# rhofield/rho-tts

Measured on AMD Instinct MI355X. Metric: audio-sec/wall-sec (RTF) Qwen3-TTS-1.7B batch=32, higher is better.
Workload: dtype bf16; 1 GPU; Qwen3-TTS-1.7B bf16, batch 32/GPU, 30-s reference clone, 10-word sentences (44 frames each), sampling=top-k 50 T 0.9, seeded synthetic weights; value counts delivered (post-processed) audio; global_batch=32, parallelism=dp1

## Files before the change

### include/rho_tts_amd_debug.h

```cpp
#ifndef RHO_TTS_AMD_DEBUG_H
#define RHO_TTS_AMD_DEBUG_H

#include "rho_tts_amd.h"

#ifdef __cplusplus
extern "C" {
#endif

RT_API int rt_profile_enable(rt_model* m, int32_t on);
RT_API int rt_profile_read(rt_model* m, int64_t* n_launches, double* total_ms, double* total_bytes);
RT_API int rt_profile_read_class(rt_model* m, int32_t cls, int64_t* n_launches, double* total_ms, double* total_bytes);

RT_API int rt_debug_gemm(rt_ctx* ctx, const void* d_a, int32_t a_is_f32, int64_t M, int32_t cin, int32_t taps, int32_t tap_stride,
                         int32_t tap_offset, int32_t rows_out, int32_t rows_in, const void* d_w_bf16, int32_t N,
                         const float* d_bias, int32_t act, float* d_out, int32_t mode, int32_t split_k);
RT_API int rt_debug_attention(rt_ctx* ctx, const float* d_q, int32_t M, int32_t heads, int32_t kv_heads, int32_t head_dim,
                              const int32_t* d_row_slot, const int32_t* d_row_pos, int32_t window, const void* d_k, const void* d_v,
                              int32_t slots, int32_t max_pos, void* d_out_bf16);
RT_API int rt_debug_attention_planes(rt_ctx* ctx, const float* d_q, int32_t M, int32_t heads, int32_t kv_heads, int32_t head_dim,
                                     const int32_t* d_row_slot, const int32_t* d_row_pos, int32_t window, const void* d_k_hi,
                                     const void* d_k_lo, const void* d_v_hi, const void* d_v_lo, int32_t slots, int32_t max_pos,
                                     float* d_out_f32);
RT_API int rt_debug_gemm_col(rt_ctx* ctx, const void* d_a_bf16, int32_t M, int32_t K, const void* d_w_bf16, int32_t N, int32_t epi, int32_t split,
                             int32_t row_off, int32_t nt, const float* d_rowsq, int32_t rowsq_n, float eps, const float* d_bias,
// ... 119 lines not shown
                             const rt_debug_epi* e2, int32_t pair_mode);

RT_API int rt_debug_enc_conv0(rt_ctx* ctx, const float* d_pcm, int64_t T, int32_t C, int32_t K, const float* d_w, const float* d_bias, float* d_x,
                              void* d_hi, void* d_lo);
RT_API int rt_debug_rvq(rt_ctx* ctx, const float* d_sem, float* d_aco, int32_t T, int32_t D, int32_t K, int32_t Q, const void* const* h_cbT,
                        int32_t* d_codes);
RT_API int rt_debug_stats_pool(rt_ctx* ctx, const float* d_x, int32_t T, int32_t C, float* d_out);
RT_API int rt_debug_gemv_f32(rt_ctx* ctx, const float* d_W, const float* d_b_or_NULL, const float* d_x, int32_t N, int32_t K, int32_t relu,
                             float* d_y);
RT_API int rt_debug_voice_encode_stages(rt_model* m, const float* h_pcm, int64_t n_samples, int32_t max_frames, float* h_feats, float* h_tf,
                                        float* h_emb, float* h_sem, float* h_aco, int32_t* h_codes, int32_t* h_n_frames,
                                        float* h_speaker_embed);

RT_API int rt_debug_tune(int32_t code, int32_t arg);
RT_API int rt_debug_col_row_blocks(int32_t n_cu, int32_t M, int32_t N, int32_t epi, int32_t split);
RT_API int rt_bench_gemm_col(rt_ctx* ctx, int32_t M, int32_t N, int32_t K, int32_t a_norm, int32_t epi, int32_t n_mats, int32_t iters,
                             double* avg_us, int64_t* stamps8);
RT_API int rt_bench_stt_gather(rt_ctx* ctx, int32_t layers, int32_t rows, int32_t heads, int32_t max_pos, int32_t head_dim, int32_t prefix, int32_t step,
                               int32_t iters, double* us_ranged, double* us_uniform);
RT_API int rt_bench_launch(rt_ctx* ctx, int32_t grid_wgs, int32_t n, int32_t use_graph, int32_t reps, double* us_per_launch);
RT_API int rt_bench_grid_barrier(rt_ctx* ctx, int32_t wgs, int32_t threads, int32_t n, int32_t mode, double* us_per_barrier, int32_t* aborted);
RT_API int rt_bench_sample(rt_ctx* ctx, const float* d_logits, int32_t M, int32_t V, const rt_sampling* sp, int32_t iters, double* avg_us,
                           int64_t* stamps8);
RT_API int rt_bench_attention_fused(rt_ctx* ctx, int32_t M, int32_t heads, int32_t kv_heads, int32_t head_dim, int32_t prefix_len, int32_t own_len,
                                    int32_t shared, int32_t layers, int32_t iters, double* avg_us);
RT_API int rt_bench_gemm_skinny(rt_ctx* ctx, int32_t M, int32_t N, int32_t K, int32_t split_k, int32_t n_mats, int32_t iters,
                                double* avg_us, int32_t* used_split);

#ifdef __cplusplus
}
// ... 3 lines not shown
```

### rho_tts_amd/csrc/debug.hip

```cpp
#include <algorithm>
#include <vector>

#include "kernels.h"

namespace {
__global__ void k_touch(float* p, int n) {
    const int i = blockIdx.x * blockDim.x + threadIdx.x;
    if (i < n) p[i] = p[i] * 1.0001f + 1.0f;
}
template <int MODE>
__global__ void k_bench_barrier(unsigned* bar, int n, float* buf) {
    const int i = blockIdx.x * blockDim.x + threadIdx.x;
    const int j = (i + blockDim.x) % (gridDim.x * blockDim.x);
    float acc = buf[i];
    for (int e = 1; e <= n; ++e) {
        if (MODE == 2) st_agent(buf + i, acc + 1.0f); else buf[i] = acc + 1.0f;
        if (!grid_barrier<MODE>(bar, gridDim.x, (unsigned)e, 1u << 20)) return;
        acc = MODE == 2 ? ld_agent(buf + j) : buf[j];
        if (acc != (float)e && i == 0) bar[2] = 1u;
    }
    buf[i] = acc;
}
template <int P>
__global__ void k_bench_pair(unsigned* flags, int n, float* buf, unsigned* bar) {
// ... 13 lines not shown
                while (__hip_atomic_load(flags + mate * 32, __ATOMIC_ACQUIRE, __HIP_MEMORY_SCOPE_AGENT) < (unsigned)e)
                    if (++spins > (1u << 22)) { bar[1] = 1u; break; }
            }
            __syncthreads();
            if (bar[1]) return;
            if (t < 512 && ld_agent(theirs + t) != (float)e) bar[2] = 1u;
        }
    }
}
__global__ void k_iota64(int64_t* p, int n) {
    const int i = blockIdx.x * blockDim.x + threadIdx.x;
    if (i < n) p[i] = i;
}

template <typename T>
__global__ void k_tile_rows(const T* __restrict__ src, int M, int K, int row_off, T* __restrict__ dst) {
    const int64_t n = (int64_t)M * K;
    for (int64_t i = (int64_t)blockIdx.x * blockDim.x + threadIdx.x; i < n; i += (int64_t)gridDim.x * blockDim.x) {
        const int m = (int)(i / K), k = (int)(i % K);
        dst[tile_off(row_off + m, k, K)] = src[i];
    }
}
template <typename T>
__global__ void k_untile_rows(const T* __restrict__ src, int M, int K, int row_off, T* __restrict__ dst) {
    const int64_t n = (int64_t)M * K;
    for (int64_t i = (int64_t)blockIdx.x * blockDim.x + threadIdx.x; i < n; i += (int64_t)gridDim.x * blockDim.x) {
        const int m = (int)(i / K), k = (int)(i % K);
        dst[i] = src[tile_off(row_off + m, k, K)];
    }
}
}

#define RT_KNOB_DEFINE(base, name, def, lo, hi, doc) rt_knob name{def};
RT_KNOBS(RT_KNOB_DEFINE)
RT_KNOB_ARG(RT_KNOB_DEFINE)
#undef RT_KNOB_DEFINE
std::atomic<int> g_tune_epoch{0};
namespace {
struct KnobRow { int base, lo, hi; rt_knob* knob; };
#define RT_KNOB_ROW(base, name, def, lo, hi, doc) {base, lo, hi, &name},
const KnobRow kKnobs[] = {RT_KNOBS(RT_KNOB_ROW)};
const KnobRow kKnobArg[] = {RT_KNOB_ARG(RT_KNOB_ROW)};
#undef RT_KNOB_ROW
// ... 82 lines not shown
}

int rt_debug_gemm_col(rt_ctx* ctx, const void* d_a_bf16, int32_t M, int32_t K, const void* d_w_bf16, int32_t N, int32_t epi, int32_t split,
                      int32_t row_off, int32_t nt, const float* d_rowsq, int32_t rowsq_n, float eps, const float* d_bias, const float* d_scale,
                      float* d_x, const float* d_next_norm_w, void* d_next_bf16, float* d_rowsq_out, void* d_act_bf16) {
    if (!ctx || !d_a_bf16 || !d_w_bf16 || M < 1 || M > 128 || K < 32 || K % 32 || N < 1 || row_off < 0 || row_off % 16)
        return rt_fail(ctx, RT_ERR_INVALID, "rt_debug_gemm_col: bad argument (1 <= M <= 128, K %% 32 == 0, row_off %% 16 == 0)");
    if (epi < COL_STORE || epi > COL_SILU) return rt_fail(ctx, RT_ERR_INVALID, "rt_debug_gemm_col: epi %d", epi);
    if ((epi != COL_SILU && !d_x) || (epi == COL_SILU && (!d_act_bf16 || N % 32)) || (epi == COL_RESID && !d_rowsq_out))
        return rt_fail(ctx, RT_ERR_INVALID, "rt_debug_gemm_col: missing output for epilogue %d", epi);
    CtxLock g(ctx);
    RT_HIP(ctx, hipSetDevice(ctx->device));
    const int No = epi == COL_SILU ? N / 2 : N;
    if (split <= 0) split = epi == COL_SILU ? col_split_silu(N, ctx->n_cu) : col_split_for(N, ctx->n_cu);
    const int rows = (row_off + M + 31) / 32 * 32;
    bf16_t *w16 = nullptr, *a_t = nullptr, *next_t = nullptr, *act_t = nullptr;
    float *x_t = nullptr, *rowsq_all = nullptr, *rowsq_out_all = nullptr;
    int rc = RT_OK;
    auto cleanup = [&]() {
        (void)hipStreamSynchronize(ctx->stream);
        for (void* p : {(void*)w16, (void*)a_t, (void*)next_t, (void*)act_t, (void*)x_t, (void*)rowsq_all, (void*)rowsq_out_all}) if (p) (void)hipFree(p);
    };
#define DBG_HIP(expr) do { hipError_t _e = (expr); if (_e != hipSuccess) { cleanup(); return rt_fail(ctx, rt_hip_status(_e), "%s failed: %s", #expr, hipGetErrorString(_e)); } } while (0)
    DBG_HIP(hipMalloc((void**)&w16, packed16_bytes(N, K)));
    DBG_HIP(hipMalloc((void**)&a_t, (size_t)rows * K * 2));
    DBG_HIP(hipMemsetAsync(a_t, 0, (size_t)rows * K * 2, ctx->stream));
    PackedW pw;
    pw.N = N; pw.K = K;
    rc = launch_pack_weight16(ctx, (const bf16_t*)d_w_bf16, N, K, w16, &pw);
    const int nb = 256;
    hipLaunchKernelGGL((k_tile_rows<bf16_t>), dim3(nb), dim3(256), 0, ctx->stream, (const bf16_t*)d_a_bf16, M, K, row_off, a_t);
    const int n_part = (N + 15) / 16 * split;
    ColArgs c;
    c.A = a_t; c.M = M; c.K = K; c.epi = epi; c.split = split; c.row_off = row_off; c.nt = nt ? 1 : 0; c.eps = eps;
    c.bias = d_bias; c.scale = d_scale; c.ldc = No;
    if (d_rowsq) {
        DBG_HIP(hipMalloc((void**)&rowsq_all, (size_t)rows * rowsq_n * 4));
        DBG_HIP(hipMemsetAsync(rowsq_all, 0, (size_t)rows * rowsq_n * 4, ctx->stream));
        DBG_HIP(hipMemcpyAsync(rowsq_all + (size_t)row_off * rowsq_n, d_rowsq, (size_t)M * rowsq_n * 4, hipMemcpyDeviceToDevice, ctx->stream));
        c.post_scale = 1; c.rowsq = rowsq_all; c.rowsq_n = rowsq_n;
    }
    if (epi == COL_STORE) {
        c.out = d_x - (size_t)row_off * No;
    } else if (epi == COL_RESID) {
        DBG_HIP(hipMalloc((void**)&x_t, (size_t)rows * No * 4));
        DBG_HIP(hipMemsetAsync(x_t, 0, (size_t)rows * No * 4, ctx->stream));
        hipLaunchKernelGGL((k_tile_rows<float>), dim3(nb), dim3(256), 0, ctx->stream, (const float*)d_x, M, No, row_off, x_t);
        DBG_HIP(hipMalloc((void**)&rowsq_out_all, (size_t)rows * n_part * 4));
        DBG_HIP(hipMemsetAsync(rowsq_out_all, 0, (size_t)rows * n_part * 4, ctx->stream));
        c.out = x_t; c.rowsq_out = rowsq_out_all; c.rowsq_out_n = n_part;
        if (d_next_bf16) {
            DBG_HIP(hipMalloc((void**)&next_t, (size_t)rows * No * 2));
            DBG_HIP(hipMemsetAsync(next_t, 0, (size_t)rows * No * 2, ctx->stream));
            c.next_bf16 = next_t; c.next_norm_w = d_next_norm_w;
        }
    } else {
        DBG_HIP(hipMalloc((void**)&act_t, (size_t)rows * No * 2));
        DBG_HIP(hipMemsetAsync(act_t, 0, (size_t)rows * No * 2, ctx->stream));
        c.out_bf16 = act_t;
    }
    const int blk = (M > 64 && g_col_rows128) ? 128 : (g_col_rows64 ? 64 : 32);
    for (int r0 = 0; r0 < M && !rc; r0 += blk) {
        ColArgs a = c;
        a.M = std::min(blk, M - r0);
        a.row_off = row_off + r0;
        rc = launch_gemm_col(ctx, a, pw);
    }
    if (!rc && epi == COL_RESID) {
        hipLaunchKernelGGL((k_untile_rows<float>), dim3(nb), dim3(256), 0, ctx->stream, (const float*)x_t, M, No, row_off, d_x);
        if (next_t) hipLaunchKernelGGL((k_untile_rows<bf16_t>), dim3(nb), dim3(256), 0, ctx->stream, (const bf16_t*)next_t, M, No, row_off, (bf16_t*)d_next_bf16);
        DBG_HIP(hipMemcpyAsync(d_rowsq_out, rowsq_out_all + (size_t)row_off * n_part, (size_t)M * n_part * 4, hipMemcpyDeviceToDevice, ctx->stream));
    }
    if (!rc && epi == COL_SILU)
        hipLaunchKernelGGL((k_untile_rows<bf16_t>), dim3(nb), dim3(256), 0, ctx->stream, (const bf16_t*)act_t, M, No, row_off, (bf16_t*)d_act_bf16);
    if (!rc) DBG_HIP(hipGetLastError());
#undef DBG_HIP
    cleanup();
    return rc;
}

int rt_debug_attention_fused(rt_ctx* ctx, const float* d_qkv, int32_t M, int32_t heads, int32_t kv_heads, int32_t head_dim, const float* d_q_norm_w,
                             const float* d_k_norm_w, float eps, const float* d_cos, const float* d_sin, const int32_t* d_row_slot,
                             const int32_t* d_row_pos, int32_t pos_add, void* d_k, void* d_v, int32_t slots, int32_t max_pos,
                             int32_t prefix_slot, int32_t prefix_len, void* d_out_bf16) {
    if (!ctx || !d_qkv || !d_cos || !d_sin || !d_k || !d_v || !d_out_bf16 || M < 1)
        return rt_fail(ctx, RT_ERR_INVALID, "rt_debug_attention_fused: null argument");
    if (prefix_slot >= slots || prefix_len < 0 || prefix_len > max_pos) return rt_fail(ctx, RT_ERR_INVALID, "rt_debug_attention_fused: bad prefix");
    CtxLock g(ctx);
    RT_HIP(ctx, hipSetDevice(ctx->device));
// ... 117 lines not shown
    RT_HIP(ctx, bufs.alloc(out, sizeof(GatherSrc) * (size_t)n_src));
    RT_HIP(ctx, hipMemcpy(*out, h.data(), sizeof(GatherSrc) * (size_t)n_src, hipMemcpyHostToDevice));
    return RT_OK;
}
int dbg_finish(rt_ctx* ctx, int rc) {
    const hipError_t se = hipStreamSynchronize(ctx->stream);
    if (rc) return rc;
    RT_HIP(ctx, se);
    return RT_OK;
}
template <typename T>
int dbg_tile_in(rt_ctx* ctx, DbgBufs& bufs, const T* rows_rm, int rows, int H, T** tiled) {
    const size_t pad = (size_t)(rows + 15) / 16 * 16;
    RT_HIP(ctx, bufs.alloc(tiled, pad * H * sizeof(T)));
    RT_HIP(ctx, hipMemsetAsync(*tiled, 0, pad * H * sizeof(T), ctx->stream));
    hipLaunchKernelGGL((k_tile_rows<T>), dim3(256), dim3(256), 0, ctx->stream, rows_rm, rows, H, 0, *tiled);
    RT_HIP(ctx, hipGetLastError());
    return RT_OK;
}
template <typename T>
int dbg_tile_out(rt_ctx* ctx, const T* tiled, int rows, int H, T* rows_rm) {
    hipLaunchKernelGGL((k_untile_rows<T>), dim3(256), dim3(256), 0, ctx->stream, tiled, rows, H, 0, rows_rm);
    RT_HIP(ctx, hipGetLastError());
    return RT_OK;
}
int dbg_read_i32(rt_ctx* ctx, const int32_t* d, int n, std::vector<int32_t>& h) {
    h.assign((size_t)n, 0);
    RT_HIP(ctx, hipStreamSynchronize(ctx->stream));
    RT_HIP(ctx, hipMemcpy(h.data(), d, (size_t)n * 4, hipMemcpyDeviceToHost));
    return RT_OK;
}
}
}

int rt_debug_add_rmsnorm(rt_ctx* ctx, float* d_x, int32_t M, int32_t H, const float* d_slabs, int32_t n_slabs, const float* d_slab_bias,
                         const float* d_scale, const float* d_w, float eps, void* d_out_bf16, float* d_out_f32) {
    if (!ctx || !d_x || M < 1 || H < 1 || n_slabs < 0 || (n_slabs > 0 && !d_slabs))
// ... 267 lines not shown
        if (code >= r.base + r.lo && code <= r.base + r.hi) {
            *r.knob = code - r.base;
            if (r.base == kKnobArg[0].base && arg >= kKnobArg[0].lo && arg <= kKnobArg[0].hi) *kKnobArg[0].knob = arg;
            ++g_tune_epoch;
            return RT_OK;
        }
    return RT_ERR_INVALID;
}

int rt_debug_col_row_blocks(int32_t n_cu, int32_t M, int32_t N, int32_t epi, int32_t split) {
    if (n_cu < 1 || M < 1 || M > 128 || N < 1 || epi < COL_STORE || epi > COL_SILU || (epi == COL_SILU && N % 32) || split > 4 || split == 3) return -1;
    std::shared_lock<std::shared_mutex> plan(g_tune_mu);
    bool x_form = false;
    const int wg = col_workgroups(n_cu, M, N, epi, split, &x_form);
    return col_row_blocks(n_cu, M, wg, x_form);
}

int rt_bench_gemm_skinny(rt_ctx* ctx, int32_t M, int32_t N, int32_t K, int32_t split_k, int32_t n_mats, int32_t iters, double* avg_us,
                         int32_t* used_split) {
    if (!ctx || !avg_us || M < 1 || M > 64 || N < 32 || K < 16 || K % 16 || n_mats < 1 || iters < 1) return rt_fail(ctx, RT_ERR_INVALID, "rt_bench_gemm_skinny: bad argument");
    CtxLock g(ctx);
    RT_HIP(ctx, hipSetDevice(ctx->device));
    const size_t pb = packed_bytes(N, K);
    bf16_t* wbuf = nullptr;
    bf16_t* a = nullptr;
    float* out = nullptr;
    if (split_k < 1) split_k = skinny_pick_split(M, N, K, ctx->n_cu);
    if (used_split) *used_split = split_k;
    RT_HIP(ctx, hipMalloc((void**)&wbuf, pb * n_mats));
    RT_HIP(ctx, hipMalloc((void**)&a, (size_t)M * K * 2));
// ... 372 lines not shown
```

### rho_tts_amd/csrc/gemm_col.hip

```cpp
#include <hip/hip_ext.h>

#include "kernels.h"

namespace {

typedef __attribute__((ext_vector_type(8))) __bf16 bf8_t;
typedef __attribute__((ext_vector_type(8))) short s8_t;
typedef __attribute__((ext_vector_type(16))) float f16_t;
typedef __attribute__((ext_vector_type(4))) float f4_t;
typedef __attribute__((ext_vector_type(4))) int i4_t;

__device__ __forceinline__ f16_t mfma32(s8_t a, s8_t b, f16_t c) {
    return __builtin_amdgcn_mfma_f32_32x32x16_bf16(__builtin_bit_cast(bf8_t, a), __builtin_bit_cast(bf8_t, b), c, 0, 0, 0);
}
__device__ __forceinline__ unsigned pk2(float lo, float hi) { return f32x2_to_bf16x2(lo, hi); }

constexpr int WAVES = 8;

typedef __attribute__((ext_vector_type(4))) float f4acc_t;
__device__ __forceinline__ f4acc_t mfma16(s8_t a, s8_t b, f4acc_t c) {
    return __builtin_amdgcn_mfma_f32_16x16x32_bf16(__builtin_bit_cast(bf8_t, a), __builtin_bit_cast(bf8_t, b), c, 0, 0, 0);
}

constexpr int col_chunk(int epi, int mt, bool x) {
    if (mt == 8) return epi == COL_SILU ? 1 : 2;
    return epi == COL_SILU ? (x ? (mt == 4 ? 2 : 4) : 2) : ((mt == 4 || mt == 1) ? 4 : 8);
}
template <int EPI, int MT, int NPRE, bool X = false, bool NORM = false, int WQ = 0, int CF = 0, bool RB = false>
__global__ __launch_bounds__(512, (((EPI == COL_SILU && MT == 2) || (MT == 1 && !RB)) && !X) ? 4 : 2) void k_gemm_col(ColArgs g) {
    static_assert(!X || (EPI == COL_SILU && MT >= 2), "the extra half pair exists for gate/up only");
    static_assert(!RB || (!X && MT <= 2), "row blocks have 16 or 32 rows, and the 1.5-pair form is never blocked");
    constexpr int RMT = MT > 4 ? 4 : MT;
    constexpr int ROUNDS = MT / RMT;
    __shared__ float red[WAVES][RMT][4][64];
    __shared__ float sh_inv[16 * MT];
    constexpr int NB = (EPI == COL_SILU) ? (X ? 3 : 2) : 1;
    static_assert(WQ == 0 || NORM, "wide requests exist for the row-scale partials only");
    static_assert(CF == 0 || (EPI != COL_SILU && (MT == 2 || (MT == 1 && RB))), "fitted chunks exist for STORE / RESID launches of up to 32 rows only");
    constexpr int C = CF ? CF : col_chunk(EPI, (RB && MT == 1) ? 2 : MT, X);
    constexpr int PASSES = (MT + 1) / 2;
    const int tid = threadIdx.x, lane = tid & 63, w = tid >> 6;
    const int r = lane & 15, qd = lane >> 4;
    const int rb0 = RB ? (int)blockIdx.y * (16 * MT) : 0;
    const int row_off = g.row_off + rb0;
    const int M = RB ? (g.M - rb0 < 16 * MT ? g.M - rb0 : 16 * MT) : g.M;
    const int sp_shift = g.split == 4 ? 2 : (g.split == 2 ? 1 : 0);
// ... 177 lines not shown
            if (ok) {
                v += e_bias;
                g.out[(int64_t)(row_off + e_row) * g.ldc + n] = v;
            }
        } else if (EPI == COL_RESID) {
            float xn = 0.f;
            if (ok) {
                v += e_bias;
                v *= e_scale;
                xn = xres[ps] + v;
                const int64_t o = tile_off(row_off + e_row, n, (int)g.ldc);
                g.out[o] = xn;
                if (g.next_bf16) g.next_bf16[o] = f32_to_bf16(e_nw * xn);
            }
            float sq = xn * xn;
            sq = group_sum_f32<16>(sq);
            if ((e_l & 15) == 0 && e_row < M) g.rowsq_out[(int64_t)(row_off + e_row) * g.rowsq_out_n + (g.rowsq_perm ? rowsq_slot((int)blockIdx.x, g.rowsq_out_n) : (int)blockIdx.x)] = sq;
        } else {
            if (ok) {
                const float u = val[1][ps] * inv;
                g.out_bf16[tile_off(row_off + e_row, n, (int)g.ldc)] = f32_to_bf16(v / (1.f + __expf(-v)) * u);
            }
            if (X) {
                const float gx = val[NB - 1][ps] * inv;
                const float ux = __shfl_down(gx, 8, 16);
                const int nx = x_tile * 16 + x_col0 + (e_l & 7);
                if (e_row < M && (e_l & 15) < 8 && nx < g.N) g.out_bf16[tile_off(row_off + e_row, nx, (int)g.ldc)] = f32_to_bf16(gx / (1.f + __expf(-gx)) * ux);
            }
        }
    }
    if (g.stamps && blockIdx.x == 0 && (!RB || blockIdx.y == 0) && tid == 0) g.stamps[5] = wall_clock64();
}

template <int EPI, int MT, int NPRE, bool X, bool NORM, int WQ, int CF, bool RB>
void launch_one(rt_ctx* ctx, const ColArgs& g, dim3 grid, hipEvent_t e0, hipEvent_t e1) {
    if (!e0 && !e1) hipLaunchKernelGGL((k_gemm_col<EPI, MT, NPRE, X, NORM, WQ, CF, RB>), grid, dim3(512), 0, ctx->stream, g);
    else hipExtLaunchKernelGGL((k_gemm_col<EPI, MT, NPRE, X, NORM, WQ, CF, RB>), grid, dim3(512), 0, ctx->stream, e0, e1, 0, g);
}

template <int EPI, int MT, bool X, bool NORM, int WQ, int CF, bool RB>
void launch_npre2(rt_ctx* ctx, const ColArgs& g, dim3 grid, hipEvent_t e0, hipEvent_t e1) {
    constexpr int C = CF ? CF : col_chunk(EPI, (RB && MT == 1) ? 2 : MT, X);
    const int kchunk = (g.KT + WAVES - 1) / WAVES;
    const bool all_waves_busy = g.KT >= WAVES && (WAVES - 1) * kchunk < g.KT;
    const int n_sc = (kchunk + C - 1) / C;
    if (!all_waves_busy) launch_one<EPI, MT, 0, X, NORM, WQ, CF, RB>(ctx, g, grid, e0, e1);
    else if (n_sc >= 2) launch_one<EPI, MT, 2, X, NORM, WQ, CF, RB>(ctx, g, grid, e0, e1);
    else launch_one<EPI, MT, 1, X, NORM, WQ, CF, RB>(ctx, g, grid, e0, e1);
}

template <int EPI, int MT, bool X, bool NORM, int WQ, bool RB>
void launch_chunk(rt_ctx* ctx, const ColArgs& g, dim3 grid, hipEvent_t e0, hipEvent_t e1) {
    if constexpr (EPI != COL_SILU && (MT == 2 || (MT == 1 && RB))) {
        const int kchunk = (g.KT + WAVES - 1) / WAVES;
        if (g_col_chunk_fit && kchunk <= 4) return launch_npre2<EPI, MT, X, NORM, WQ, 4, RB>(ctx, g, grid, e0, e1);
        if (g_col_chunk_fit && kchunk > 8 && kchunk <= 12) return launch_npre2<EPI, MT, X, NORM, WQ, 6, RB>(ctx, g, grid, e0, e1);
    }
    launch_npre2<EPI, MT, X, NORM, WQ, 0, RB>(ctx, g, grid, e0, e1);
}

template <int EPI, int MT, bool X = false, bool RB = false>
void launch_npre(rt_ctx* ctx, const ColArgs& g, dim3 grid, hipEvent_t e0, hipEvent_t e1) {
    if (g.post_scale) {
        if constexpr (EPI != COL_RESID) {
            if (g.rowsq_wide == 2) launch_chunk<EPI, MT, X, true, 2, RB>(ctx, g, grid, e0, e1);
            else if (g.rowsq_wide == 4) launch_chunk<EPI, MT, X, true, 4, RB>(ctx, g, grid, e0, e1);
            else launch_chunk<EPI, MT, X, true, 0, RB>(ctx, g, grid, e0, e1);
        }
    } else {
        launch_chunk<EPI, MT, X, false, 0, RB>(ctx, g, grid, e0, e1);
    }
}

int dispatch_epi(rt_ctx* ctx, const ColArgs& g, dim3 grid, hipEvent_t e0, hipEvent_t e1) {
    if (g.row_block) {
        const bool b32 = g.row_block == 32;
        switch (g.epi) {
            case COL_STORE: b32 ? launch_npre<COL_STORE, 2, false, true>(ctx, g, grid, e0, e1) : launch_npre<COL_STORE, 1, false, true>(ctx, g, grid, e0, e1); break;
            case COL_RESID: b32 ? launch_npre<COL_RESID, 2, false, true>(ctx, g, grid, e0, e1) : launch_npre<COL_RESID, 1, false, true>(ctx, g, grid, e0, e1); break;
            case COL_SILU: b32 ? launch_npre<COL_SILU, 2, false, true>(ctx, g, grid, e0, e1) : launch_npre<COL_SILU, 1, false, true>(ctx, g, grid, e0, e1); break;
            default: return rt_fail(ctx, RT_ERR_INVALID, "gemm_col: bad epilogue %d", g.epi);
        }
        RT_HIP(ctx, hipGetLastError());
        return RT_OK;
    }
    const bool wide = g.M > 32, narrow = g.M <= 16 && g_col_rows16;
    if (g.M > 64) {
        switch (g.epi) {
            case COL_STORE: launch_npre<COL_STORE, 8>(ctx, g, grid, e0, e1); break;
            case COL_RESID: launch_npre<COL_RESID, 8>(ctx, g, grid, e0, e1); break;
            case COL_SILU:
                if (g.x_tile0 > 0) launch_npre<COL_SILU, 8, true>(ctx, g, grid, e0, e1);
                else launch_npre<COL_SILU, 8>(ctx, g, grid, e0, e1);
                break;
// ... 38 lines not shown
    }
    if (split <= 0) split = col_split_silu(N, n_cu);
    const int tiles = (N + 15) / 16 / 2;
    const int wg = tiles / 3 * 2;
    const bool narrow = M <= 16 && g_col_rows16;
    if (g_col_silu_x && split == 1 && !narrow && tiles % 3 == 0 && tiles > n_cu && wg <= n_cu && (N / 2) % 16 == 0) {
        if (x_form) *x_form = true;
        return wg;
    }
    return tiles * split;
}

int col_row_blocks(int n_cu, int M, int wg, bool x_form) {
    const int v = g_col_row_blocks;
    if (x_form || v < 1 || wg < 1 || 2 * wg > n_cu) return 0;
    if (M >= 33 && M <= 64) return 32;
    if (v >= 2 && M >= 17 && M <= 32) return 16;
    return 0;
}

bool rowsq_permuted(int n) { return g_rowsq_wide && n % 64 == 0 && n >= 64 && n <= 256; }

int launch_gemm_col(rt_ctx* ctx, const ColArgs& a, const PackedW& w, hipEvent_t ev_start, hipEvent_t ev_stop) {
    if (a.M < 1 || a.M > 128) return rt_fail(ctx, RT_ERR_INVALID, "gemm_col: M=%d outside 1..128 (callers split larger row blocks)", a.M);
    if (w.K != a.K || w.K % 32) return rt_fail(ctx, RT_ERR_INVALID, "gemm_col: K mismatch (%d vs %d) or not a multiple of 32", w.K, a.K);
    if (!w.data16) return rt_fail(ctx, RT_ERR_STATE, "gemm_col: weight has no 16-column decode copy");
    ColArgs g = a;
    g.Wp = w.data16;
    g.NT = w.Np16 / 16;
    g.KT = w.K / 32;
// ... 12 lines not shown
            tiles = wg;
        }
    } else {
        g.N = w.N;
    }
    if (wg != tiles * g.split) return rt_fail(ctx, RT_ERR_STATE, "gemm_col: %d workgroups planned, %d x %d tiles", wg, tiles, g.split);
    if (g.epi == COL_RESID && (!g.rowsq_out || g.rowsq_out_n < g.NT * g.split)) return rt_fail(ctx, RT_ERR_INVALID, "gemm_col: rowsq_out too small");
    if (g.post_scale && (!g.rowsq || g.rowsq_n < 1)) return rt_fail(ctx, RT_ERR_INVALID, "gemm_col: row scaling without partials");
    if (g.post_scale && g.epi == COL_RESID) return rt_fail(ctx, RT_ERR_UNSUPPORTED, "gemm_col: the residual epilogue has no row-scaled instantiation");
    if (g.next_bf16 && !g.next_norm_w) return rt_fail(ctx, RT_ERR_INVALID, "gemm_col: next operand without its norm weight");
    g.rowsq_perm = (g.epi == COL_RESID && rowsq_permuted(g.rowsq_out_n)) ? 1 : 0;
    g.rowsq_wide = (g.post_scale && rowsq_permuted(g.rowsq_n)) ? (g.rowsq_n <= 128 ? 2 : 4) : 0;
    if (g.rowsq_wide && (reinterpret_cast<uintptr_t>(g.rowsq) & 15))
        return rt_fail(ctx, RT_ERR_INVALID, "gemm_col: rowsq rows read in 16-byte pieces must be 16-byte aligned");
    g.row_block = col_row_blocks(ctx->n_cu, g.M, wg, x_form);
    const int n_blocks = g.row_block ? (g.M + g.row_block - 1) / g.row_block : 1;
    return dispatch_epi(ctx, g, dim3(wg, n_blocks), ev_start, ev_stop);
}
```

### rho_tts_amd/csrc/kernels.h

```cpp
#pragma once
#include "common.h"
#include "knobs.h"

struct PackedW {
    const bf16_t* data = nullptr;
    int N = 0, K = 0;
    int Np = 0, Kp = 0;
    size_t bytes() const { return (size_t)Np * Kp * 2; }
    const bf16_t* data16 = nullptr;
    int Np16 = 0;
};

struct GemmA {
    const void* ptr = nullptr;
    const void* ptr_lo = nullptr;
    int is_f32 = 0;
    int split = 0;
    int64_t M = 0;
    int Cin = 0;
    int taps = 1;
    int tap_stride = 1;
    int tap_offset = 0;
    int rows_out = 0;
    int rows_in = 0;
// ... 54 lines not shown
    bf16_t* next_bf16 = nullptr;
    const float* next_norm_w = nullptr;
    int64_t ldc = 0;
    const float* bias = nullptr;
    const float* scale = nullptr;
    float* rowsq_out = nullptr;
    int rowsq_out_n = 0;
    bf16_t* out_bf16 = nullptr;
    long long* stamps = nullptr;
    const bf16_t* Wp = nullptr;
    int NT = 0, KT = 0, N = 0, up_tile_offset = 0;
    int x_tile0 = 0;
    int rowsq_perm = 0;
    int rowsq_wide = 0;
    int row_block = 0;
};
int col_row_blocks(int n_cu, int M, int wg, bool x_form);
int col_workgroups(int n_cu, int M, int N, int epi, int split, bool* x_form);
bool rowsq_permuted(int n);
int launch_gemm_col(rt_ctx* ctx, const ColArgs& a, const PackedW& w, hipEvent_t ev_start = nullptr, hipEvent_t ev_stop = nullptr);
struct RowsqGather {
    const float* table = nullptr;
    const int32_t* idx = nullptr;
    int idx_stride = 1, first = 0;
    const int32_t* frame_ptr = nullptr;
    int64_t idx_frame_stride = 0;
};
int launch_rowsq(rt_ctx* ctx, const float* x, int M, int H, float* rowsq, int rowsq_n, float* x_tiled = nullptr,
                 bf16_t* a_tiled = nullptr, const float* norm_w = nullptr, const int32_t* src_rows = nullptr,
                 const int32_t* dst_rows = nullptr, const RowsqGather* gather = nullptr);

struct GatherSrc;
// ... 136 lines not shown
```

### rho_tts_amd/csrc/knobs.h

```cpp
#pragma once
#include "common.h"

#define RT_KNOBS(X) \
    X(0, g_skinny_variant, 0, 0, 2, "legacy skinny GEMM: 0 k_gemm_skinny, 1 k_gemm_skinny2<.,4>, 2 k_gemm_skinny2<.,8>") \
    X(100, g_decode_col, 1, 0, 1, "0 legacy 9-launch split-K decode, 1 column-owner GEMM + fused attention (5 launches per layer)") \
    X(200, g_use_graph, 1, 0, 1, "0 eager decode frames, 1 replayed from captured hipGraphs") \
    X(300, g_pred_nt, 0, 0, 1, "predictor weights: 0 cacheable loads (Infinity-Cache resident across its 15 passes), 1 non-temporal") \
    X(400, g_decode_lanes, 1, 1, 8, "decode lanes: groups of items decoding concurrently on their own streams (rt_generate)") \
    X(500, g_col_split, 0, 0, 4, "sub-tile split of narrow decode GEMMs: 0 automatic (col_split_for), 1 / 2 / 4 forced") \
    X(600, g_tile96, 1, 0, 1, "1: 128x96 workgroup tiles for N = 96 / 192 (codec decoder), 0: always 128x128") \
    X(700, g_col_rows64, 1, 0, 1, "1: one 64-row decode GEMM launch for the predictor's two-position pass, 0: two 32-row launches") \
    X(800, g_fuse_sample_embed, 1, 0, 1, "1: sampler + next-input embedding in one launch (predictor groups), 0: separate k_embed_rowsq") \
    X(900, g_prefill_fill, 3, 0, 99, "workgroups per CU a prefill GEMM's split-K aims for") \
    X(1000, g_xcd_order, 1, 0, 1, "1: tiled GEMMs run a row tile's column tiles back to back on one XCD") \
    X(1100, g_final_conv, 1, 0, 1, "the codec decoder's last conv: 1 its own LDS-window kernel, 0 a one-column GEMM") \
    X(1200, g_conv_win, 1, 0, 1, "1: k>1 convs on operand planes keep their input window in LDS (k_conv_win), 0: per-tap kernel") \
    X(1300, g_sync_parts, 0, 0, 1, "1: rt_generate waits for the stream after every frame part (bounds the dispatches in flight; profiling aid)") \
    X(1400, g_eos_check_every, 8, 1, 99, "frames between two host looks at the device-side end-of-sequence flags (1 = every frame)") \
    X(1500, g_attn_mfma, 0, 0, 2, "the talker's shared-prefix decode attention: 0 vector unit, 1 / 2 matrix cores with four rows / one row per workgroup (attention_mfma.hip); 1 measured " \
        "16.6 us per launch against 13.3 us for the vector-unit kernel at batch 32 / 460 prefix rows, so off") \
    X(1600, g_col_split4, 0, 0, 1, "1: the automatic split may go to quarter tiles (N <= 1024 on 256 CUs); measured 1.4 ms/step slower than half tiles") \
    X(1700, g_handover_every, 4, 1, 99, "queued items (n_items > rows): frames between two looks at the flags + row hand-overs.  Measured on the 1.7B model, 512 / 64 ragged texts on 32 " \
        "rows: 2 -> 487 / 445, 3 -> 489 / 445, 4 -> 491 / 447, 6 -> 485 / 445, 8 -> 477 / 428, 12 -> 475 / 434 audio-s/s (a hand-over costs ~1.4 ms, a waiting row 0.13 ms per frame)") \
    X(1800, g_conv_tall, 1, 0, 2, "k>1 convs of the 96- / 192-channel stages: 0 128-row tiles, 1 256-row tiles for long inputs, 2 always") \
// ... 12 lines not shown
    X(3000, g_fuse_conv192, 1, 0, 1, "1: the 192-channel conv pairs fuse as well, weight fragments staged through LDS") \
    X(3100, g_pred_qkv_table, 1, 0, 1, "predictor passes 2..G-1: 1 layer 0's q/k/v row of the drawn code is copied from the table rt_model_finalize builds (by the launch " \
        "that embeds the code), 0 the layer-0 qkv GEMM launch runs (same bits either way)") \
    X(3200, g_col_rows128, 1, 0, 1, "generations on 65..128 rows: 1 one 128-row decode GEMM launch per weight matrix (k_gemm_col MT = 8: the weights are streamed once), " \
        "0 two 64-row launches (same bits either way).  Measured (1.7B, profiles/r18_rows128.txt): bench.py --corpus 512 --batch 128 1014 audio-s/s with 1 against 887 with 0 (five alternating pairs; 824 on 64 rows); " \
        "per launch at 128 rows qkv 13.7 / 16.3 us, o 12.0 / 14.2, gate/up 20.9 / 27.4, down 27.3 / 29.7 (one launch / two)") \
    X(3300, g_stt_gather_ranged, 1, 0, 1, "speech-to-text under a prompt policy, the gather between beam steps: 1 the ranged form (generated positions only; the prefix " \
        "sits in both caches), 0 the uniform form over [0, longest prefix of the group + step) (same bits either way; profiles/r20_stt_prompt.txt)") \
    X(3400, g_rowsq_wide, 1, 0, 1, "RMSNorm sum-of-squares partials of the decode GEMMs, rows of n partials with n % 64 == 0 and n <= 256: 1 stored permuted (rowsq_slot) " \
        "and fetched by the row-scale prologue in 2 / 4 16-byte requests per lane, 0 stored plainly and fetched in 16 dword requests (same bits either way; " \
        "profiles/r21_gemm_col_prologue.txt)") \
    X(3500, g_col_chunk_fit, 1, 0, 1, "STORE / RESID decode GEMM launches of up to 32 rows: 1 the chunk length follows the wave's run of k-tiles (one chunk of 4 for K <= 1024, " \
        "two of 6 for K = 3072: no clamped re-loads of the run's last tile), 0 chunks of 8 (same bits either way; profiles/r21_gemm_col_prologue.txt)") \
    X(3600, g_col_row_blocks, 2, 0, 2, "decode GEMM launches whose workgroups fill at most half of the CUs (the predictor's o / down / mtp: 128 on 256) deal their rows over " \
        "gridDim.y: 0 never, 1 launches of 33..64 rows as two 32-row blocks, 2 also launches of 17..32 rows as two 16-row blocks (same bits either way; " \
        "profiles/r24_row_blocks.txt)")

#define RT_KNOB_ARG(X) \
    X(0, g_skinny_waves_per_cu, 4, 1, 0x7fffffff, "legacy skinny GEMM: split-K is chosen so that about this many waves per CU stream weights")

#define RT_KNOB_EXTERN(base, name, def, lo, hi, doc) extern rt_knob name;
RT_KNOBS(RT_KNOB_EXTERN)
RT_KNOB_ARG(RT_KNOB_EXTERN)
#undef RT_KNOB_EXTERN
extern std::atomic<int> g_tune_epoch;
```

Before: 609.2 audio-s/s.

## Deal rows over gridDim.y for split-2 STORE/RESID decode GEMMs instead of half-tiles

Split-2 STORE/RESID decode GEMM launches, whose half-tile workgroups fill more than half the CUs (talker o/down, predictor head), now run whole-tile workgroups with split 1. Their rows are dealt over gridDim.y in 32- or 16-row blocks. This keeps the workgroup count the same while each CU streams fewer weight bytes through L1. The RESID epilogue gets an HP variant that writes two half-tile rowsq partials, so downstream consumers still see the split-2 layout. The debug tile helpers gain a leading-dimension argument, and a query function for the new plan is added.

```diff
diff --git a/include/rho_tts_amd_debug.h b/include/rho_tts_amd_debug.h
--- a/include/rho_tts_amd_debug.h
+++ b/include/rho_tts_amd_debug.h
@@ -157,6 +157,7 @@
 
 RT_API int rt_debug_tune(int32_t code, int32_t arg);
 RT_API int rt_debug_col_row_blocks(int32_t n_cu, int32_t M, int32_t N, int32_t epi, int32_t split);
+RT_API int rt_debug_col_tile_blocks(int32_t n_cu, int32_t M, int32_t N, int32_t epi, int32_t split);
 RT_API int rt_bench_gemm_col(rt_ctx* ctx, int32_t M, int32_t N, int32_t K, int32_t a_norm, int32_t epi, int32_t n_mats, int32_t iters,
                              double* avg_us, int64_t* stamps8);
 RT_API int rt_bench_stt_gather(rt_ctx* ctx, int32_t layers, int32_t rows, int32_t heads, int32_t max_pos, int32_t head_dim, int32_t prefix, int32_t step,
diff --git a/rho_tts_amd/csrc/debug.hip b/rho_tts_amd/csrc/debug.hip
--- a/rho_tts_amd/csrc/debug.hip
+++ b/rho_tts_amd/csrc/debug.hip
@@ -51,19 +51,19 @@
 }
 
 template <typename T>
-__global__ void k_tile_rows(const T* __restrict__ src, int M, int K, int row_off, T* __restrict__ dst) {
+__global__ void k_tile_rows(const T* __restrict__ src, int M, int K, int row_off, T* __restrict__ dst, int ld) {
     const int64_t n = (int64_t)M * K;
     for (int64_t i = (int64_t)blockIdx.x * blockDim.x + threadIdx.x; i < n; i += (int64_t)gridDim.x * blockDim.x) {
         const int m = (int)(i / K), k = (int)(i % K);
-        dst[tile_off(row_off + m, k, K)] = src[i];
+        dst[tile_off(row_off + m, k, ld)] = src[i];
     }
 }
 template <typename T>
-__global__ void k_untile_rows(const T* __restrict__ src, int M, int K, int row_off, T* __restrict__ dst) {
+__global__ void k_untile_rows(const T* __restrict__ src, int M, int K, int row_off, T* __restrict__ dst, int ld) {
     const int64_t n = (int64_t)M * K;
     for (int64_t i = (int64_t)blockIdx.x * blockDim.x + threadIdx.x; i < n; i += (int64_t)gridDim.x * blockDim.x) {
         const int m = (int)(i / K), k = (int)(i % K);
-        dst[i] = src[tile_off(row_off + m, k, K)];
+        dst[i] = src[tile_off(row_off + m, k, ld)];
     }
 }
 }
@@ -176,6 +176,7 @@
     const int No = epi == COL_SILU ? N / 2 : N;
     if (split <= 0) split = epi == COL_SILU ? col_split_silu(N, ctx->n_cu) : col_split_for(N, ctx->n_cu);
     const int rows = (row_off + M + 31) / 32 * 32;
+    const int ldt = (No + 31) / 32 * 32;
     bf16_t *w16 = nullptr, *a_t = nullptr, *next_t = nullptr, *act_t = nullptr;
     float *x_t = nullptr, *rowsq_all = nullptr, *rowsq_out_all = nullptr;
     int rc = RT_OK;
@@ -191,11 +192,11 @@
     pw.N = N; pw.K = K;
     rc = launch_pack_weight16(ctx, (const bf16_t*)d_w_bf16, N, K, w16, &pw);
     const int nb = 256;
-    hipLaunchKernelGGL((k_tile_rows<bf16_t>), dim3(nb), dim3(256), 0, ctx->stream, (const bf16_t*)d_a_bf16, M, K, row_off, a_t);
+    hipLaunchKernelGGL((k_tile_rows<bf16_t>), dim3(nb), dim3(256), 0, ctx->stream, (const bf16_t*)d_a_bf16, M, K, row_off, a_t, K);
     const int n_part = (N + 15) / 16 * split;
     ColArgs c;
     c.A = a_t; c.M = M; c.K = K; c.epi = epi; c.split = split; c.row_off = row_off; c.nt = nt ? 1 : 0; c.eps = eps;
-    c.bias = d_bias; c.scale = d_scale; c.ldc = No;
+    c.bias = d_bias; c.scale = d_scale; c.ldc = epi == COL_STORE ? No : ldt;
     if (d_rowsq) {
         DBG_HIP(hipMalloc((void**)&rowsq_all, (size_t)rows * rowsq_n * 4));
         DBG_HIP(hipMemsetAsync(rowsq_all, 0, (size_t)rows * rowsq_n * 4, ctx->stream));
@@ -205,20 +206,20 @@
     if (epi == COL_STORE) {
         c.out = d_x - (size_t)row_off * No;
     } else if (epi == COL_RESID) {
-        DBG_HIP(hipMalloc((void**)&x_t, (size_t)rows * No * 4));
-        DBG_HIP(hipMemsetAsync(x_t, 0, (size_t)rows * No * 4, ctx->stream));
-        hipLaunchKernelGGL((k_tile_rows<float>), dim3(nb), dim3(256), 0, ctx->stream, (const float*)d_x, M, No, row_off, x_t);
+        DBG_HIP(hipMalloc((void**)&x_t, (size_t)rows * ldt * 4));
+        DBG_HIP(hipMemsetAsync(x_t, 0, (size_t)rows * ldt * 4, ctx->stream));
+        hipLaunchKernelGGL((k_tile_rows<float>), dim3(nb), dim3(256), 0, ctx->stream, (const float*)d_x, M, No, row_off, x_t, ldt);
         DBG_HIP(hipMalloc((void**)&rowsq_out_all, (size_t)rows * n_part * 4));
         DBG_HIP(hipMemsetAsync(rowsq_out_all, 0, (size_t)rows * n_part * 4, ctx->stream));
         c.out = x_t; c.rowsq_out = rowsq_out_all; c.rowsq_out_n = n_part;
         if (d_next_bf16) {
-            DBG_HIP(hipMalloc((void**)&next_t, (size_t)rows * No * 2));
-            DBG_HIP(hipMemsetAsync(next_t, 0, (size_t)rows * No * 2, ctx->stream));
+            DBG_HIP(hipMalloc((void**)&next_t, (size_t)rows * ldt * 2));
+            DBG_HIP(hipMemsetAsync(next_t, 0, (size_t)rows * ldt * 2, ctx->stream));
             c.next_bf16 = next_t; c.next_norm_w = d_next_norm_w;
         }
     } else {
-        DBG_HIP(hipMalloc((void**)&act_t, (size_t)rows * No * 2));
-        DBG_HIP(hipMemsetAsync(act_t, 0, (size_t)rows * No * 2, ctx->stream));
+        DBG_HIP(hipMalloc((void**)&act_t, (size_t)rows * ldt * 2));
+        DBG_HIP(hipMemsetAsync(act_t, 0, (size_t)rows * ldt * 2, ctx->stream));
         c.out_bf16 = act_t;
     }
     const int blk = (M > 64 && g_col_rows128) ? 128 : (g_col_rows64 ? 64 : 32);
@@ -229,12 +230,12 @@
         rc = launch_gemm_col(ctx, a, pw);
     }
     if (!rc && epi == COL_RESID) {
-        hipLaunchKernelGGL((k_untile_rows<float>), dim3(nb), dim3(256), 0, ctx->stream, (const float*)x_t, M, No, row_off, d_x);
-        if (next_t) hipLaunchKernelGGL((k_untile_rows<bf16_t>), dim3(nb), dim3(256), 0, ctx->stream, (const bf16_t*)next_t, M, No, row_off, (bf16_t*)d_next_bf16);
+        hipLaunchKernelGGL((k_untile_rows<float>), dim3(nb), dim3(256), 0, ctx->stream, (const float*)x_t, M, No, row_off, d_x, ldt);
+        if (next_t) hipLaunchKernelGGL((k_untile_rows<bf16_t>), dim3(nb), dim3(256), 0, ctx->stream, (const bf16_t*)next_t, M, No, row_off, (bf16_t*)d_next_bf16, ldt);
         DBG_HIP(hipMemcpyAsync(d_rowsq_out, rowsq_out_all + (size_t)row_off * n_part, (size_t)M * n_part * 4, hipMemcpyDeviceToDevice, ctx->stream));
     }
     if (!rc && epi == COL_SILU)
-        hipLaunchKernelGGL((k_untile_rows<bf16_t>), dim3(nb), dim3(256), 0, ctx->stream, (const bf16_t*)act_t, M, No, row_off, (bf16_t*)d_act_bf16);
+        hipLaunchKernelGGL((k_untile_rows<bf16_t>), dim3(nb), dim3(256), 0, ctx->stream, (const bf16_t*)act_t, M, No, row_off, (bf16_t*)d_act_bf16, ldt);
     if (!rc) DBG_HIP(hipGetLastError());
 #undef DBG_HIP
     cleanup();
@@ -382,13 +383,13 @@
     const size_t pad = (size_t)(rows + 15) / 16 * 16;
     RT_HIP(ctx, bufs.alloc(tiled, pad * H * sizeof(T)));
     RT_HIP(ctx, hipMemsetAsync(*tiled, 0, pad * H * sizeof(T), ctx->stream));
-    hipLaunchKernelGGL((k_tile_rows<T>), dim3(256), dim3(256), 0, ctx->stream, rows_rm, rows, H, 0, *tiled);
+    hipLaunchKernelGGL((k_tile_rows<T>), dim3(256), dim3(256), 0, ctx->stream, rows_rm, rows, H, 0, *tiled, H);
     RT_HIP(ctx, hipGetLastError());
     return RT_OK;
 }
 template <typename T>
 int dbg_tile_out(rt_ctx* ctx, const T* tiled, int rows, int H, T* rows_rm) {
-    hipLaunchKernelGGL((k_untile_rows<T>), dim3(256), dim3(256), 0, ctx->stream, tiled, rows, H, 0, rows_rm);
+    hipLaunchKernelGGL((k_untile_rows<T>), dim3(256), dim3(256), 0, ctx->stream, tiled, rows, H, 0, rows_rm, H);
     RT_HIP(ctx, hipGetLastError());
     return RT_OK;
 }
@@ -686,6 +687,16 @@
     bool x_form = false;
     const int wg = col_workgroups(n_cu, M, N, epi, split, &x_form);
     return col_row_blocks(n_cu, M, wg, x_form);
+}
+
+int rt_debug_col_tile_blocks(int32_t n_cu, int32_t M, int32_t N, int32_t epi, int32_t split) {
+    if (n_cu < 1 || M < 1 || M > 128 || N < 1 || epi < COL_STORE || epi > COL_SILU || (epi == COL_SILU && N % 32) || split > 4 || split == 3) return -1;
+    std::shared_lock<std::shared_mutex> plan(g_tune_mu);
+    if (epi == COL_SILU) return 0;
+    if (split <= 0) split = col_split_for(N, n_cu);
+    bool x_form = false;
+    if (col_row_blocks(n_cu, M, col_workgroups(n_cu, M, N, epi, split, &x_form), x_form)) return 0;
+    return col_tile_blocks(n_cu, M, (N + 15) / 16, epi, split);
 }
 
 int rt_bench_gemm_skinny(rt_ctx* ctx, int32_t M, int32_t N, int32_t K, int32_t split_k, int32_t n_mats, int32_t iters, double* avg_us,
diff --git a/rho_tts_amd/csrc/gemm_col.hip b/rho_tts_amd/csrc/gemm_col.hip
--- a/rho_tts_amd/csrc/gemm_col.hip
+++ b/rho_tts_amd/csrc/gemm_col.hip
@@ -26,10 +26,11 @@
     if (mt == 8) return epi == COL_SILU ? 1 : 2;
     return epi == COL_SILU ? (x ? (mt == 4 ? 2 : 4) : 2) : ((mt == 4 || mt == 1) ? 4 : 8);
 }
-template <int EPI, int MT, int NPRE, bool X = false, bool NORM = false, int WQ = 0, int CF = 0, bool RB = false>
+template <int EPI, int MT, int NPRE, bool X = false, bool NORM = false, int WQ = 0, int CF = 0, bool RB = false, bool HP = false>
 __global__ __launch_bounds__(512, (((EPI == COL_SILU && MT == 2) || (MT == 1 && !RB)) && !X) ? 4 : 2) void k_gemm_col(ColArgs g) {
     static_assert(!X || (EPI == COL_SILU && MT >= 2), "the extra half pair exists for gate/up only");
     static_assert(!RB || (!X && MT <= 2), "row blocks have 16 or 32 rows, and the 1.5-pair form is never blocked");
+    static_assert(!HP || (RB && EPI == COL_RESID), "two half-tile partials per workgroup exist for row-blocked RESID launches only");
     constexpr int RMT = MT > 4 ? 4 : MT;
     constexpr int ROUNDS = MT / RMT;
     __shared__ float red[WAVES][RMT][4][64];
@@ -237,8 +238,14 @@
                 if (g.next_bf16) g.next_bf16[o] = f32_to_bf16(e_nw * xn);
             }
             float sq = xn * xn;
-            sq = group_sum_f32<16>(sq);
-            if ((e_l & 15) == 0 && e_row < M) g.rowsq_out[(int64_t)(row_off + e_row) * g.rowsq_out_n + (g.rowsq_perm ? rowsq_slot((int)blockIdx.x, g.rowsq_out_n) : (int)blockIdx.x)] = sq;
+            if constexpr (HP) {
+                sq = group_sum_f32<8>(sq);
+                const int j = 2 * nt + ((e_l >> 3) & 1);
+                if ((e_l & 7) == 0 && e_row < M) g.rowsq_out[(int64_t)(row_off + e_row) * g.rowsq_out_n + (g.rowsq_perm ? rowsq_slot(j, g.rowsq_out_n) : j)] = sq;
+            } else {
+                sq = group_sum_f32<16>(sq);
+                if ((e_l & 15) == 0 && e_row < M) g.rowsq_out[(int64_t)(row_off + e_row) * g.rowsq_out_n + (g.rowsq_perm ? rowsq_slot((int)blockIdx.x, g.rowsq_out_n) : (int)blockIdx.x)] = sq;
+            }
         } else {
             if (ok) {
                 const float u = val[1][ps] * inv;
@@ -255,43 +262,43 @@
     if (g.stamps && blockIdx.x == 0 && (!RB || blockIdx.y == 0) && tid == 0) g.stamps[5] = wall_clock64();
 }
 
-template <int EPI, int MT, int NPRE, bool X, bool NORM, int WQ, int CF, bool RB>
+template <int EPI, int MT, int NPRE, bool X, bool NORM, int WQ, int CF, bool RB, bool HP>
 void launch_one(rt_ctx* ctx, const ColArgs& g, dim3 grid, hipEvent_t e0, hipEvent_t e1) {
-    if (!e0 && !e1) hipLaunchKernelGGL((k_gemm_col<EPI, MT, NPRE, X, NORM, WQ, CF, RB>), grid, dim3(512), 0, ctx->stream, g);
-    else hipExtLaunchKernelGGL((k_gemm_col<EPI, MT, NPRE, X, NORM, WQ, CF, RB>), grid, dim3(512), 0, ctx->stream, e0, e1, 0, g);
-}
-
-template <int EPI, int MT, bool X, bool NORM, int WQ, int CF, bool RB>
+    if (!e0 && !e1) hipLaunchKernelGGL((k_gemm_col<EPI, MT, NPRE, X, NORM, WQ, CF, RB, HP>), grid, dim3(512), 0, ctx->stream, g);
+    else hipExtLaunchKernelGGL((k_gemm_col<EPI, MT, NPRE, X, NORM, WQ, CF, RB, HP>), grid, dim3(512), 0, ctx->stream, e0, e1, 0, g);
+}
+
+template <int EPI, int MT, bool X, bool NORM, int WQ, int CF, bool RB, bool HP>
 void launch_npre2(rt_ctx* ctx, const ColArgs& g, dim3 grid, hipEvent_t e0, hipEvent_t e1) {
     constexpr int C = CF ? CF : col_chunk(EPI, (RB && MT == 1) ? 2 : MT, X);
     const int kchunk = (g.KT + WAVES - 1) / WAVES;
     const bool all_waves_busy = g.KT >= WAVES && (WAVES - 1) * kchunk < g.KT;
     const int n_sc = (kchunk + C - 1) / C;
-    if (!all_waves_busy) launch_one<EPI, MT, 0, X, NORM, WQ, CF, RB>(ctx, g, grid, e0, e1);
-    else if (n_sc >= 2) launch_one<EPI, MT, 2, X, NORM, WQ, CF, RB>(ctx, g, grid, e0, e1);
-    else launch_one<EPI, MT, 1, X, NORM, WQ, CF, RB>(ctx, g, grid, e0, e1);
-}
-
-template <int EPI, int MT, bool X, bool NORM, int WQ, bool RB>
+    if (!all_waves_busy) launch_one<EPI, MT, 0, X, NORM, WQ, CF, RB, HP>(ctx, g, grid, e0, e1);
+    else if (n_sc >= 2) launch_one<EPI, MT, 2, X, NORM, WQ, CF, RB, HP>(ctx, g, grid, e0, e1);
+    else launch_one<EPI, MT, 1, X, NORM, WQ, CF, RB, HP>(ctx, g, grid, e0, e1);
+}
+
+template <int EPI, int MT, bool X, bool NORM, int WQ, bool RB, bool HP>
 void launch_chunk(rt_ctx* ctx, const ColArgs& g, dim3 grid, hipEvent_t e0, hipEvent_t e1) {
     if constexpr (EPI != COL_SILU && (MT == 2 || (MT == 1 && RB))) {
         const int kchunk = (g.KT + WAVES - 1) / WAVES;
-        if (g_col_chunk_fit && kchunk <= 4) return launch_npre2<EPI, MT, X, NORM, WQ, 4, RB>(ctx, g, grid, e0, e1);
-        if (g_col_chunk_fit && kchunk > 8 && kchunk <= 12) return launch_npre2<EPI, MT, X, NORM, WQ, 6, RB>(ctx, g, grid, e0, e1);
-    }
-    launch_npre2<EPI, MT, X, NORM, WQ, 0, RB>(ctx, g, grid, e0, e1);
-}
-
-template <int EPI, int MT, bool X = false, bool RB = false>
+        if (g_col_chunk_fit && kchunk <= 4) return launch_npre2<EPI, MT, X, NORM, WQ, 4, RB, HP>(ctx, g, grid, e0, e1);
+        if (g_col_chunk_fit && kchunk > 8 && kchunk <= 12) return launch_npre2<EPI, MT, X, NORM, WQ, 6, RB, HP>(ctx, g, grid, e0, e1);
+    }
+    launch_npre2<EPI, MT, X, NORM, WQ, 0, RB, HP>(ctx, g, grid, e0, e1);
+}
+
+template <int EPI, int MT, bool X = false, bool RB = false, bool HP = false>
 void launch_npre(rt_ctx* ctx, const ColArgs& g, dim3 grid, hipEvent_t e0, hipEvent_t e1) {
     if (g.post_scale) {
         if constexpr (EPI != COL_RESID) {
-            if (g.rowsq_wide == 2) launch_chunk<EPI, MT, X, true, 2, RB>(ctx, g, grid, e0, e1);
-            else if (g.rowsq_wide == 4) launch_chunk<EPI, MT, X, true, 4, RB>(ctx, g, grid, e0, e1);
-            else launch_chunk<EPI, MT, X, true, 0, RB>(ctx, g, grid, e0, e1);
+            if (g.rowsq_wide == 2) launch_chunk<EPI, MT, X, true, 2, RB, HP>(ctx, g, grid, e0, e1);
+            else if (g.rowsq_wide == 4) launch_chunk<EPI, MT, X, true, 4, RB, HP>(ctx, g, grid, e0, e1);
+            else launch_chunk<EPI, MT, X, true, 0, RB, HP>(ctx, g, grid, e0, e1);
         }
     } else {
-        launch_chunk<EPI, MT, X, false, 0, RB>(ctx, g, grid, e0, e1);
+        launch_chunk<EPI, MT, X, false, 0, RB, HP>(ctx, g, grid, e0, e1);
     }
 }
 
@@ -300,7 +307,10 @@
         const bool b32 = g.row_block == 32;
         switch (g.epi) {
             case COL_STORE: b32 ? launch_npre<COL_STORE, 2, false, true>(ctx, g, grid, e0, e1) : launch_npre<COL_STORE, 1, false, true>(ctx, g, grid, e0, e1); break;
-            case COL_RESID: b32 ? launch_npre<COL_RESID, 2, false, true>(ctx, g, grid, e0, e1) : launch_npre<COL_RESID, 1, false, true>(ctx, g, grid, e0, e1); break;
+            case COL_RESID:
+                if (g.lay_split != g.split) b32 ? launch_npre<COL_RESID, 2, false, true, true>(ctx, g, grid, e0, e1) : launch_npre<COL_RESID, 1, false, true, true>(ctx, g, grid, e0, e1);
+                else b32 ? launch_npre<COL_RESID, 2, false, true>(ctx, g, grid, e0, e1) : launch_npre<COL_RESID, 1, false, true>(ctx, g, grid, e0, e1);
+                break;
             case COL_SILU: b32 ? launch_npre<COL_SILU, 2, false, true>(ctx, g, grid, e0, e1) : launch_npre<COL_SILU, 1, false, true>(ctx, g, grid, e0, e1); break;
             default: return rt_fail(ctx, RT_ERR_INVALID, "gemm_col: bad epilogue %d", g.epi);
         }
@@ -369,6 +379,14 @@
 int col_row_blocks(int n_cu, int M, int wg, bool x_form) {
     const int v = g_col_row_blocks;
     if (x_form || v < 1 || wg < 1 || 2 * wg > n_cu) return 0;
+    if (M >= 33 && M <= 64) return 32;
+    if (v >= 2 && M >= 17 && M <= 32) return 16;
+    return 0;
+}
+
+int col_tile_blocks(int n_cu, int M, int tiles, int epi, int split) {
+    const int v = g_col_tile_blocks;
+    if (v < 1 || (epi != COL_STORE && epi != COL_RESID) || split != 2 || tiles < 1 || tiles * 2 > n_cu || 2 * tiles * 2 <= n_cu) return 0;
     if (M >= 33 && M <= 64) return 32;
     if (v >= 2 && M >= 17 && M <= 32) return 16;
     return 0;
@@ -411,6 +429,15 @@
     if (g.rowsq_wide && (reinterpret_cast<uintptr_t>(g.rowsq) & 15))
         return rt_fail(ctx, RT_ERR_INVALID, "gemm_col: rowsq rows read in 16-byte pieces must be 16-byte aligned");
     g.row_block = col_row_blocks(ctx->n_cu, g.M, wg, x_form);
+    g.lay_split = g.split;
+    int wg_x = wg;
+    if (!g.row_block && !x_form) {
+        g.row_block = col_tile_blocks(ctx->n_cu, g.M, tiles, g.epi, g.split);
+        if (g.row_block) {
+            g.split = 1;
+            wg_x = tiles;
+        }
+    }
     const int n_blocks = g.row_block ? (g.M + g.row_block - 1) / g.row_block : 1;
-    return dispatch_epi(ctx, g, dim3(wg, n_blocks), ev_start, ev_stop);
-}
+    return dispatch_epi(ctx, g, dim3(wg_x, n_blocks), ev_start, ev_stop);
+}
diff --git a/rho_tts_amd/csrc/kernels.h b/rho_tts_amd/csrc/kernels.h
--- a/rho_tts_amd/csrc/kernels.h
+++ b/rho_tts_amd/csrc/kernels.h
@@ -92,8 +92,10 @@
     int rowsq_perm = 0;
     int rowsq_wide = 0;
     int row_block = 0;
+    int lay_split = 0;
 };
 int col_row_blocks(int n_cu, int M, int wg, bool x_form);
+int col_tile_blocks(int n_cu, int M, int tiles, int epi, int split);
 int col_workgroups(int n_cu, int M, int N, int epi, int split, bool* x_form);
 bool rowsq_permuted(int n);
 int launch_gemm_col(rt_ctx* ctx, const ColArgs& a, const PackedW& w, hipEvent_t ev_start = nullptr, hipEvent_t ev_stop = nullptr);
diff --git a/rho_tts_amd/csrc/knobs.h b/rho_tts_amd/csrc/knobs.h
--- a/rho_tts_amd/csrc/knobs.h
+++ b/rho_tts_amd/csrc/knobs.h
@@ -50,7 +50,11 @@
         "two of 6 for K = 3072: no clamped re-loads of the run's last tile), 0 chunks of 8 (same bits either way; profiles/r21_gemm_col_prologue.txt)") \
     X(3600, g_col_row_blocks, 2, 0, 2, "decode GEMM launches whose workgroups fill at most half of the CUs (the predictor's o / down / mtp: 128 on 256) deal their rows over " \
         "gridDim.y: 0 never, 1 launches of 33..64 rows as two 32-row blocks, 2 also launches of 17..32 rows as two 16-row blocks (same bits either way; " \
-        "profiles/r24_row_blocks.txt)")
+        "profiles/r24_row_blocks.txt)") \
+    X(3700, g_col_tile_blocks, 2, 0, 2, "STORE / RESID decode GEMM launches at split 2 whose half-tile workgroups fill more than half of the CUs (the 1.7B talker's o / down, the " \
+        "predictor's head: N = 2048, 256 workgroups of 32 rows x 8 columns) run whole-tile workgroups with their rows dealt over gridDim.y - as many workgroups, fewer bytes into " \
+        "each CU's L1: 0 never, 1 launches of 33..64 rows as 32-row blocks, 2 also launches of 17..32 rows as 16-row blocks (same bits either way, the rowsq row keeps its " \
+        "split-2 layout; profiles/r25_tile_blocks.txt)")
 
 #define RT_KNOB_ARG(X) \
     X(0, g_skinny_waves_per_cu, 4, 1, 0x7fffffff, "legacy skinny GEMM: split-K is chosen so that about this many waves per CU stream weights")
```

Result: faster. 619.7 audio-s/s (median of 6 runs) (+1.7%).
